# mayuelala/FollowYourClick

Measured on AMD Instinct MI355X. Metric: denoised frames/sec, 16f x 512^2 clip @ 25 DDIM steps, higher is better.
Workload: dtype bf16; 1 GPU; configs[1]: AnimationPipeline DDIM loop, SD-1.5 UNet3D + mm_sd_v15-shaped motion modules (random init), 1 clip/GPU of 16 frames 512x512, 25 DDIM steps, CFG 8.0, mask + first-frame concat, fps/flow conditioning; frames=16, height=512, width=512, ddim_steps=25, parallelism=dp1 (independent clips, weight broadcast 0.00 GiB in 0.00s)

## Files before the change

followyourclick_amd/csrc/attention.hip:

```cpp
#include "attention_kernel.h"

extern "C" int fyc_attention(const fyc_attn_args* a, void* stream) {
  FYC_REQUIRE(a && a->q && a->k && a->vt && a->o, "fyc_attention: null pointer");
  FYC_REQUIRE(g_fyc_zero_page != nullptr, "fyc_attention: fyc_init() not called");
  FYC_REQUIRE(a->dtype == FYC_BF16 || a->dtype == FYC_F16, "fyc_attention: bf16 / f16 only (f32 parity mode uses materialised attention)");
  FYC_REQUIRE(a->batch > 0 && a->heads > 0 && a->n_q > 0 && a->n_k > 0, "fyc_attention: bad sizes");
  FYC_REQUIRE(a->d % 8 == 0 && a->d >= 8 && a->d <= 160, "fyc_attention: head dim %d (multiple of 8, <= 160)", a->d);
  FYC_REQUIRE(a->ldvt % 8 == 0 && a->ldvt >= a->n_k, "fyc_attention: ldvt=%d must be a multiple of 8 and >= n_k", a->ldvt);
  FYC_REQUIRE(a->ldo % 4 == 0, "fyc_attention: ldo must be a multiple of 4");
  FYC_REQUIRE(a->kv_batch_div >= 1, "fyc_attention: kv_batch_div");
  FYC_REQUIRE(a->q_batch_mod >= 0 && a->q_batch_mod <= a->batch, "fyc_attention: q_batch_mod %d (0 .. batch)", a->q_batch_mod);
  fyca::AttnP p;
  p.q = (const bf16_t*)a->q; p.k = (const bf16_t*)a->k; p.vt = (const bf16_t*)a->vt; p.o = (bf16_t*)a->o;
  p.batch = a->batch; p.heads = a->heads; p.n_q = a->n_q; p.n_k = a->n_k; p.d = a->d; p.ldo = a->ldo; p.ldvt = a->ldvt;
  p.kv_batch_div = a->kv_batch_div; p.o_accumulate = a->o_accumulate; p.q_batch_mod = a->q_batch_mod;
  p.sl2e = a->scale * 1.44269504088896340736f; p.o_scale = a->o_scale;
  p.nqb = 0; p.zero = (const char*)g_fyc_zero_page;
  hipStream_t st = (hipStream_t)stream;
  const long long wg3 = (long long)a->batch * a->heads * ((a->n_q + 191) / 192);
  int qt = (a->n_q >= 1024 && wg3 >= 512 && a->d <= 48) ? 3 : 2;
  if (g_fyc_tuning[3] >= 2 && g_fyc_tuning[3] <= 4 && (a->d <= 80 || g_fyc_tuning[3] == 2)) qt = g_fyc_tuning[3];
  if (a->dtype == FYC_F16) {
    if (a->d <= 48) return fyca::run_small<f16_t>(p, qt, st);
    if (a->d <= 96) return fyca::run_medium<f16_t>(p, qt, st);
    return fyca::run_large<f16_t>(p, st);
  }
  if (a->d <= 48) return fyca::run_small<bf16_t>(p, qt, st);
  if (a->d <= 96) return fyca::run_medium<bf16_t>(p, qt, st);
  return fyca::run_large<bf16_t>(p, st);
}
```

followyourclick_amd/csrc/attention_kernel.h:

```cpp
#pragma once
#include <type_traits>

#include "fyc_common.h"

namespace fyca {

struct AttnP {
  const bf16_t* q; const bf16_t* k; const bf16_t* vt; bf16_t* o;
  int batch, heads, n_q, n_k, d, ldo, ldvt, kv_batch_div, o_accumulate;
  int q_batch_mod;
  float sl2e, o_scale;
  int nqb;
  const char* zero;
};

#define FYC_1 0x3F80
static __device__ __attribute__((aligned(16))) const unsigned short fyc_ones[72] = {
    FYC_1, FYC_1, FYC_1, FYC_1, FYC_1, FYC_1, FYC_1, FYC_1, FYC_1, FYC_1, FYC_1, FYC_1, FYC_1, FYC_1, FYC_1, FYC_1,
    FYC_1, FYC_1, FYC_1, FYC_1, FYC_1, FYC_1, FYC_1, FYC_1, FYC_1, FYC_1, FYC_1, FYC_1, FYC_1, FYC_1, FYC_1, FYC_1,
    FYC_1, FYC_1, FYC_1, FYC_1, FYC_1, FYC_1, FYC_1, FYC_1, FYC_1, FYC_1, FYC_1, FYC_1, FYC_1, FYC_1, FYC_1, FYC_1,
    FYC_1, FYC_1, FYC_1, FYC_1, FYC_1, FYC_1, FYC_1, FYC_1, FYC_1, FYC_1, FYC_1, FYC_1, FYC_1, FYC_1, FYC_1, FYC_1,
    FYC_1, 0, 0, 0, 0, 0, 0, 0};
#undef FYC_1
#define FYC_1 0x3C00
static __device__ __attribute__((aligned(16))) const unsigned short fyc_ones_f16[72] = {
    FYC_1, FYC_1, FYC_1, FYC_1, FYC_1, FYC_1, FYC_1, FYC_1, FYC_1, FYC_1, FYC_1, FYC_1, FYC_1, FYC_1, FYC_1, FYC_1,
    FYC_1, FYC_1, FYC_1, FYC_1, FYC_1, FYC_1, FYC_1, FYC_1, FYC_1, FYC_1, FYC_1, FYC_1, FYC_1, FYC_1, FYC_1, FYC_1,
    FYC_1, FYC_1, FYC_1, FYC_1, FYC_1, FYC_1, FYC_1, FYC_1, FYC_1, FYC_1, FYC_1, FYC_1, FYC_1, FYC_1, FYC_1, FYC_1,
    FYC_1, FYC_1, FYC_1, FYC_1, FYC_1, FYC_1, FYC_1, FYC_1, FYC_1, FYC_1, FYC_1, FYC_1, FYC_1, FYC_1, FYC_1, FYC_1,
    FYC_1, 0, 0, 0, 0, 0, 0, 0};
#undef FYC_1
template <typename T> __device__ __forceinline__ const unsigned short* ones_table();
template <> __device__ __forceinline__ const unsigned short* ones_table<bf16_t>() { return fyc_ones; }
template <> __device__ __forceinline__ const unsigned short* ones_table<f16_t>() { return fyc_ones_f16; }

typedef __attribute__((ext_vector_type(4))) short s16x4;

template <typename T> struct AttnMma;
template <> struct AttnMma<bf16_t> {
  __device__ static __forceinline__ f32x4 k32(bf16x8 a, bf16x8 b, f32x4 c) { return __builtin_amdgcn_mfma_f32_16x16x32_bf16(a, b, c, 0, 0, 0); }
  __device__ static __forceinline__ f32x4 k16(s16x4 a, s16x4 b, f32x4 c) { return __builtin_amdgcn_mfma_f32_16x16x16bf16_1k(a, b, c, 0, 0, 0); }
};
template <> struct AttnMma<f16_t> {
  __device__ static __forceinline__ f32x4 k32(f16x8 a, f16x8 b, f32x4 c) { return __builtin_amdgcn_mfma_f32_16x16x32_f16(a, b, c, 0, 0, 0); }
  __device__ static __forceinline__ f32x4 k16(s16x4 a, s16x4 b, f32x4 c) {
    return __builtin_amdgcn_mfma_f32_16x16x16f16(__builtin_bit_cast(f16x4, a), __builtin_bit_cast(f16x4, b), c, 0, 0, 0);
  }
};

__device__ __forceinline__ void glds16(const void* gsrc, char* lds_wave_base) {
  __builtin_amdgcn_global_load_lds((const __attribute__((address_space(1))) void*)gsrc,
                                   (__attribute__((address_space(3))) void*)lds_wave_base, 16, 0, 0);
}
template <int N> __device__ __forceinline__ void wait_vmcnt() { asm volatile("s_waitcnt vmcnt(%0)" ::"n"(N) : "memory"); }

#ifndef FYC_ATTN_BUILTIN_ISSUE
__device__ __forceinline__ void dma4_masked(unsigned long long m0_, unsigned long long m1_, unsigned long long m2_, unsigned long long m3_,
                                            unsigned o0, unsigned o1, unsigned o2, unsigned o3,
                                            const char* b0, const char* b1, const char* b2, const char* b3,
                                            unsigned l0, unsigned l1, unsigned l2, unsigned l3) {
  unsigned keep_m0;
  unsigned long long keep_exec;
  asm volatile("s_mov_b32 %[km0], m0\n\ts_mov_b64 %[kex], exec\n\t"
               "s_mov_b64 exec, %[ma]\n\ts_cbranch_execz 1f\n\ts_mov_b32 m0, %[la]\n\ts_nop 0\n\tglobal_load_lds_dwordx4 %[oa], %[ba]\n"
               "1:\n\ts_mov_b64 exec, %[mb]\n\ts_cbranch_execz 2f\n\ts_mov_b32 m0, %[lb]\n\ts_nop 0\n\tglobal_load_lds_dwordx4 %[ob], %[bb]\n"
               "2:\n\ts_mov_b64 exec, %[mc]\n\ts_cbranch_execz 3f\n\ts_mov_b32 m0, %[lc]\n\ts_nop 0\n\tglobal_load_lds_dwordx4 %[oc], %[bc]\n"
               "3:\n\ts_mov_b64 exec, %[md]\n\ts_cbranch_execz 4f\n\ts_mov_b32 m0, %[ld]\n\ts_nop 0\n\tglobal_load_lds_dwordx4 %[od], %[bd]\n"
               "4:\n\ts_mov_b64 exec, %[kex]\n\ts_mov_b32 m0, %[km0]"
               : [km0] "=&s"(keep_m0), [kex] "=&s"(keep_exec)
               : [ma] "s"(m0_), [mb] "s"(m1_), [mc] "s"(m2_), [md] "s"(m3_), [oa] "v"(o0), [ob] "v"(o1), [oc] "v"(o2), [od] "v"(o3),
                 [ba] "s"(b0), [bb] "s"(b1), [bc] "s"(b2), [bd] "s"(b3), [la] "s"(l0), [lb] "s"(l1), [lc] "s"(l2), [ld] "s"(l3)
               : "memory");
}
#endif

#ifdef FYC_ATTN_SETPRIO
#define FYC_ATTN_PRIO(x) __builtin_amdgcn_s_setprio(x)
#else
#define FYC_ATTN_PRIO(x) do { } while (0)
#endif

constexpr float RESCALE_THR = 6.0f;

__device__ __forceinline__ float quad_max(float mx) {
  mx = fmaxf(mx, __builtin_bit_cast(float, __builtin_amdgcn_ds_swizzle(__builtin_bit_cast(int, mx), 0x401F)));
  return swap32_max(mx);
}

template <typename T, int DP16, int DVT, int QT>
__global__ void __launch_bounds__(256, (DP16 == 3 && DVT == 3 && QT == 3) ? 3 : 1) fyc_attn_kernel(const AttnP p) {
  typedef typename Pair16<T>::Vec8 Frag;
  const unsigned short* const fyc_ones = ones_table<T>();
  constexpr int KS = DP16 / 2;
  constexpr bool TAIL = (DP16 & 1) != 0;
  constexpr bool MSUB = (DVT == DP16);
  constexpr bool PIPE = DP16 <= 3;
  constexpr int DC = DP16 * 2;
  constexpr bool KXOR = (DC == 8);
  constexpr int PC = KXOR ? 8 : DC + 1;
  constexpr int KB = 64;
  constexpr int K_IT = (KB * PC + 255) / 256, K_BYTES = K_IT * 256 * 16;
  constexpr int V_ROWS = DVT * 16, V_IT = (V_ROWS * 8 + 255) / 256, V_BYTES = V_IT * 256 * 16;
  constexpr int STAGE = K_BYTES + V_BYTES, LOADS = K_IT + V_IT, NS = 3;
  extern __shared__ __attribute__((aligned(16))) char smem[];

  const int tid = threadIdx.x, lane = tid & 63;
  const int wave = __builtin_amdgcn_readfirstlane(tid >> 6);
  const int g = lane >> 4, r16 = lane & 15;

  const int BH = p.batch * p.heads;
  int bh, qb;
  if ((BH & 7) == 0) {
    const int xcd = blockIdx.x & 7, j = blockIdx.x >> 3;
    bh = (j / p.nqb) * 8 + xcd;
    qb = j % p.nqb;
  } else {
    bh = blockIdx.x / p.nqb;
    qb = blockIdx.x % p.nqb;
  }
  const int b = bh / p.heads, h = bh - b * p.heads;
  const int kvb = (b / p.kv_batch_div) * p.heads + h;
  const int bh_q = p.q_batch_mod > 0 ? (b % p.q_batch_mod) * p.heads + h : bh;
  const T* Q = reinterpret_cast<const T*>(p.q) + (long long)bh_q * p.n_q * p.d;
  const T* K = reinterpret_cast<const T*>(p.k) + (long long)kvb * p.n_k * p.d;
  const T* VT = reinterpret_cast<const T*>(p.vt) + (long long)kvb * p.d * p.ldvt;
  const char* zero = p.zero;
  const int ntiles = (p.n_k + KB - 1) / KB;
  const int dchunks = p.d >> 3;

  constexpr bool OFFS_IN_LDS = (K_IT + V_IT) <= 4;
  constexpr unsigned NODATA = 0xffffffffu;
  unsigned k_off[K_IT], v_off[V_IT];
  int my_loads = 0;
#pragma unroll
  for (int it = 0; it < K_IT; ++it) {
    const int L = it * 256 + tid, row = L / PC, cc = L - row * PC;
    const int c = KXOR ? (cc ^ (row & 7)) : cc;
    k_off[it] = (row < KB && c < dchunks) ? (unsigned)(row * p.d + c * 8) * 2u : NODATA;
    my_loads += __builtin_amdgcn_ballot_w64(k_off[it] != NODATA) != 0 ? 1 : 0;
  }
#pragma unroll
  for (int it = 0; it < V_IT; ++it) {
    const int L = it * 256 + tid, row = L >> 3, cc = L & 7;
    const int c = cc ^ (row & 7);
    v_off[it] = (row < p.d) ? (unsigned)(row * p.ldvt + c * 8) * 2u : NODATA;
    my_loads += __builtin_amdgcn_ballot_w64(v_off[it] != NODATA) != 0 ? 1 : 0;
  }
  my_loads = __builtin_amdgcn_readfirstlane(my_loads);
#ifndef FYC_ATTN_BUILTIN_ISSUE
  unsigned long long dmask[4] = {0ull, 0ull, 0ull, 0ull};
  if (K_IT + V_IT <= 4) {
#pragma unroll
    for (int it = 0; it < K_IT; ++it) dmask[it] = __builtin_amdgcn_ballot_w64(k_off[it] != NODATA);
#pragma unroll
    for (int it = 0; it < V_IT; ++it) dmask[K_IT + it] = __builtin_amdgcn_ballot_w64(v_off[it] != NODATA);
  }
  const unsigned lds_ring = (unsigned)(size_t)(__attribute__((address_space(3))) char*)smem;
#endif
  char* const offs_lds = smem + NS * STAGE + tid * 16;
  if (OFFS_IN_LDS) {
    u32x4 o4 = {NODATA, NODATA, NODATA, NODATA};
#pragma unroll
    for (int it = 0; it < K_IT; ++it) o4[it] = k_off[it];
#pragma unroll
    for (int it = 0; it < V_IT; ++it) o4[K_IT + it] = v_off[it];
    *reinterpret_cast<u32x4*>(offs_lds) = o4;
  }
  auto issue_const = [&](int stage) {
    char* sK = smem + stage * STAGE;
    char* sV = sK + K_BYTES;
#pragma unroll
    for (int it = 0; it < K_IT; ++it) {
      const int L = it * 256 + tid, row = L / PC, cc = L - row * PC;
      const int c = KXOR ? (cc ^ (row & 7)) : cc;
      if (k_off[it] == NODATA) glds16((MSUB && row < KB && c == dchunks) ? (const void*)(fyc_ones + 64) : (const void*)zero, sK + (it * 256 + wave * 64) * 16);
    }
#pragma unroll
    for (int it = 0; it < V_IT; ++it) {
      const int row = (it * 256 + tid) >> 3;
      if (v_off[it] == NODATA) glds16(row == p.d ? (const void*)fyc_ones : (const void*)zero, sV + (it * 256 + wave * 64) * 16);
    }
  };
  auto issue_full = [&](int tile, int stage) {
    char* sK = smem + stage * STAGE;
    char* sV = sK + K_BYTES;
    const char* kb = reinterpret_cast<const char*>(K) + (long long)tile * (KB * 2) * p.d;
    const char* vb = reinterpret_cast<const char*>(VT) + (long long)tile * (KB * 2);
#ifndef FYC_ATTN_BUILTIN_ISSUE
    if constexpr (OFFS_IN_LDS) {
      const u32x4 o4 = *reinterpret_cast<const u32x4*>(offs_lds);
      const unsigned lk = lds_ring + stage * STAGE + wave * 1024, lv = lk + K_BYTES;
      auto base = [&](int i) { return i < K_IT ? kb : vb; };
      auto ldst = [&](int i) { return i < K_IT ? lk + i * 4096 : lv + (i - K_IT) * 4096; };
      dma4_masked(dmask[0], dmask[1], dmask[2], dmask[3], o4[0], o4[1], o4[2], o4[3], base(0), base(1), base(2), base(3), ldst(0), ldst(1), ldst(2), ldst(3));
      return;
    }
#endif
    unsigned ko[K_IT], vo[V_IT];
    if (OFFS_IN_LDS) {
      const u32x4 o4 = *reinterpret_cast<const u32x4*>(offs_lds);
#pragma unroll
      for (int it = 0; it < K_IT; ++it) ko[it] = o4[it];
#pragma unroll
      for (int it = 0; it < V_IT; ++it) vo[it] = o4[K_IT + it];
    } else {
#pragma unroll
      for (int it = 0; it < K_IT; ++it) ko[it] = k_off[it];
#pragma unroll
      for (int it = 0; it < V_IT; ++it) vo[it] = v_off[it];
    }
#pragma unroll
    for (int it = 0; it < K_IT; ++it)
      if (ko[it] != NODATA) glds16(kb + ko[it], sK + (it * 256 + wave * 64) * 16);
#pragma unroll
    for (int it = 0; it < V_IT; ++it)
      if (vo[it] != NODATA) glds16(vb + vo[it], sV + (it * 256 + wave * 64) * 16);
  };
  auto issue_general = [&](int tile, int stage) {
    char* sK = smem + stage * STAGE;
    char* sV = sK + K_BYTES;
    const int key0 = tile * KB;
#pragma unroll
    for (int it = 0; it < K_IT; ++it) {
      const int L = it * 256 + tid, row = L / PC, cc = L - row * PC;
      const int c = KXOR ? (cc ^ (row & 7)) : cc;
      const int key = key0 + row;
      const bool live = row < KB && key < p.n_k;
      const void* src = zero;
      if (live && c < dchunks) src = K + (long long)key * p.d + c * 8;
      else if (MSUB && live && c == dchunks) src = fyc_ones + 64;
      glds16(src, sK + (it * 256 + wave * 64) * 16);
    }
#pragma unroll
    for (int it = 0; it < V_IT; ++it) {
      const int L = it * 256 + tid, row = L >> 3, cc = L & 7;
      const int c = cc ^ (row & 7);
      const int key = key0 + c * 8;
      const void* src = zero;
      if (row < p.d) { if (key < p.ldvt) src = VT + (long long)row * p.ldvt + key; }
      else if (row == p.d) src = fyc_ones;
      glds16(src, sV + (it * 256 + wave * 64) * 16);
    }
  };
  const int nfull = p.n_k / KB;
  auto issue = [&](int tile, int stage) { if (tile < nfull) issue_full(tile, stage); else issue_general(tile, stage); };
  auto loads_of = [&](int tile) { return tile < nfull ? my_loads : LOADS; };
  auto wait_dyn = [&](int n) {
    switch (n) {
      case 0: wait_vmcnt<0>(); break;   case 1: wait_vmcnt<1>(); break;   case 2: wait_vmcnt<2>(); break;   case 3: wait_vmcnt<3>(); break;
      case 4: wait_vmcnt<4>(); break;   case 5: wait_vmcnt<5>(); break;   case 6: wait_vmcnt<6>(); break;   case 7: wait_vmcnt<7>(); break;
      case 8: wait_vmcnt<8>(); break;   case 9: wait_vmcnt<9>(); break;   case 10: wait_vmcnt<10>(); break; case 11: wait_vmcnt<11>(); break;
      default: wait_vmcnt<12>(); break;
    }
  };
  static_assert(LOADS <= 12, "wait_dyn covers up to 12 DMA instructions per tile");
#pragma unroll
  for (int st = 0; st < NS; ++st) issue_const(st);
  issue(0, 0);
  if (ntiles > 1) issue(1, 1);

  const int qbase = qb * (64 * QT) + wave * (16 * QT);
  Frag qf[QT][KS > 0 ? KS : 1];
  s16x4 qt4[QT];
#pragma unroll
  for (int qt = 0; qt < QT; ++qt) {
    const int query = qbase + qt * 16 + r16;
    const bool qok = query < p.n_q;
#pragma unroll
    for (int ks = 0; ks < KS; ++ks) {
      const int dd = 32 * ks + 8 * g;
      float v[8];
      load8<T>((qok && dd < p.d) ? Q + (long long)query * p.d + dd : reinterpret_cast<const T*>(zero), v);
      u32x4 pk;
#pragma unroll
      for (int i = 0; i < 4; ++i) pk[i] = Pair16<T>::pack(v[2 * i] * p.sl2e, v[2 * i + 1] * p.sl2e);
      qf[qt][ks] = __builtin_bit_cast(Frag, pk);
    }
    if (TAIL) {
      const int dd = 32 * KS + 4 * g;
      float v[4];
      ElemIO<T>::ld4((qok && dd < p.d) ? Q + (long long)query * p.d + dd : reinterpret_cast<const T*>(zero), v);
      u32x2 pk = {Pair16<T>::pack(v[0] * p.sl2e, v[1] * p.sl2e), Pair16<T>::pack(v[2] * p.sl2e, v[3] * p.sl2e)};
      qt4[qt] = __builtin_bit_cast(s16x4, pk);
    }
  }
  constexpr int MOFF = MSUB ? ((DP16 * 16 - 8) - (TAIL ? 32 * KS : 32 * (KS - 1))) : 0;
  constexpr int MG = TAIL ? MOFF / 4 : MOFF / 8;
  auto set_neg_max = [&](int qt, float m_bf16_exact) {
    const unsigned short bits = Pair16<T>::to_bits(-m_bf16_exact);
    if (g == MG) {
      if (TAIL) qt4[qt][0] = (short)bits;
      else {
        u32x4 t = __builtin_bit_cast(u32x4, qf[qt][KS > 0 ? KS - 1 : 0]);
        t[0] = (t[0] & 0xffff0000u) | bits;
        qf[qt][KS > 0 ? KS - 1 : 0] = __builtin_bit_cast(Frag, t);
      }
    }
  };

  f32x4 o[QT][DVT];
  float m_run[QT];
#pragma unroll
  for (int qt = 0; qt < QT; ++qt) {
    m_run[qt] = 0.f;
#pragma unroll
    for (int dv = 0; dv < DVT; ++dv) o[qt][dv] = (f32x4){0.f, 0.f, 0.f, 0.f};
  }
  bool started = false;

  int st_c = 0, st_i = (ntiles > 1) ? 2 : 1;
  auto tile_body = [&](const int tile, auto steady_c) __attribute__((always_inline)) {
    constexpr bool STEADY = decltype(steady_c)::value;
    if (STEADY && my_loads == LOADS) wait_vmcnt<LOADS>();
    else if (STEADY) wait_dyn(my_loads);
    else wait_dyn(tile + 1 < ntiles ? loads_of(tile + 1) : 0);
    __builtin_amdgcn_s_barrier();
    if (STEADY) { issue_full(tile + 2, st_i); st_i = (st_i + 1 == NS) ? 0 : st_i + 1; }
    else if (tile + 2 < ntiles) { issue(tile + 2, st_i); st_i = (st_i + 1 == NS) ? 0 : st_i + 1; }
    const char* sK = smem + st_c * STAGE;
    const char* sV = sK + K_BYTES;
    st_c = (st_c + 1 == NS) ? 0 : st_c + 1;
    const bool tail = STEADY ? false : (tile * KB + KB > p.n_k);
    auto qk = [&](int kb, f32x4 (&s)[2][QT]) {
      const char* kr[2];
#pragma unroll
      for (int t = 0; t < 2; ++t) kr[t] = sK + (kb * 32 + 8 * (r16 >> 2) + 4 * t + (r16 & 3)) * (PC * 16);
      s16x4 kt4[2];
      if (TAIL) {
#pragma unroll
        for (int t = 0; t < 2; ++t) {
          const int krow = kb * 32 + 8 * (r16 >> 2) + 4 * t + (r16 & 3);
          const int chunk = 4 * KS + (g >> 1);
          kt4[t] = *reinterpret_cast<const s16x4*>(kr[t] + (KXOR ? (chunk ^ (krow & 7)) : chunk) * 16 + (g & 1) * 8);
        }
      }
      FYC_ATTN_PRIO(1);
#pragma unroll
      for (int t = 0; t < 2; ++t)
#pragma unroll
        for (int qt = 0; qt < QT; ++qt) {
          s[t][qt] = (f32x4){0.f, 0.f, 0.f, 0.f};
          if (TAIL) s[t][qt] = AttnMma<T>::k16(kt4[t], qt4[qt], s[t][qt]);
        }
      if (TAIL && KS > 0) __builtin_amdgcn_sched_barrier(0);
#pragma unroll
      for (int t = 0; t < 2; ++t) {
        const int krow = kb * 32 + 8 * (r16 >> 2) + 4 * t + (r16 & 3);
        Frag kf[KS > 0 ? KS : 1];
#pragma unroll
        for (int ks = 0; ks < KS; ++ks) {
          const int chunk = 4 * ks + g;
          kf[ks] = *reinterpret_cast<const Frag*>(kr[t] + (KXOR ? (chunk ^ (krow & 7)) : chunk) * 16);
        }
#pragma unroll
        for (int qt = 0; qt < QT; ++qt)
#pragma unroll
          for (int ks = 0; ks < KS; ++ks) s[t][qt] = AttnMma<T>::k32(kf[ks], qf[qt][ks], s[t][qt]);
      }
      FYC_ATTN_PRIO(0);
    };
    auto softmax_pv = [&](int kb, f32x4 (&s)[2][QT], f32x4 (&sn)[2][QT], bool has_next) {
      float mx[QT];
#pragma unroll
      for (int qt = 0; qt < QT; ++qt) {
        if (tail) {
#pragma unroll
          for (int t = 0; t < 2; ++t)
#pragma unroll
            for (int r = 0; r < 4; ++r)
              if (tile * KB + kb * 32 + 8 * g + 4 * t + r >= p.n_k) s[t][qt][r] = -INFINITY;
        }
        const float m0 = fmaxf(fmaxf(s[0][qt][0], s[0][qt][1]), s[0][qt][2]);
        const float m1 = fmaxf(fmaxf(s[0][qt][3], s[1][qt][0]), s[1][qt][1]);
        mx[qt] = fmaxf(fmaxf(m0, m1), fmaxf(s[1][qt][2], s[1][qt][3]));
      }
      bool move = !started;
#pragma unroll
      for (int qt = 0; qt < QT; ++qt) move = move || (MSUB ? mx[qt] > RESCALE_THR : mx[qt] > m_run[qt] + RESCALE_THR);
      float shift[QT];
#pragma unroll
      for (int qt = 0; qt < QT; ++qt) shift[qt] = MSUB ? 0.f : m_run[qt];
      if (__builtin_amdgcn_ballot_w64(move) != 0) {
#pragma unroll
        for (int qt = 0; qt < QT; ++qt) mx[qt] = quad_max(mx[qt]);
#pragma unroll
        for (int qt = 0; qt < QT; ++qt) {
          const bool mv = !started || (MSUB ? mx[qt] > RESCALE_THR : mx[qt] > m_run[qt] + RESCALE_THR);
          if (MSUB) {
            const float m_new = mv ? round_through<T>(m_run[qt] + mx[qt]) : m_run[qt];
            const float delta = m_new - m_run[qt];
            const float alpha = started ? __builtin_amdgcn_exp2f(-delta) : 1.0f;
            m_run[qt] = m_new;
            shift[qt] = delta;
            set_neg_max(qt, m_new);
            if (has_next) {
#pragma unroll
              for (int t = 0; t < 2; ++t)
#pragma unroll
                for (int r = 0; r < 4; ++r) sn[t][qt][r] -= delta;
            }
#pragma unroll
            for (int dv = 0; dv < DVT; ++dv) { o[qt][dv][0] *= alpha; o[qt][dv][1] *= alpha; o[qt][dv][2] *= alpha; o[qt][dv][3] *= alpha; }
          } else {
            const float m_new = mv ? mx[qt] : m_run[qt];
            const float alpha = started ? __builtin_amdgcn_exp2f(m_run[qt] - m_new) : 1.0f;
            m_run[qt] = m_new;
            shift[qt] = m_new;
#pragma unroll
            for (int dv = 0; dv < DVT; ++dv) { o[qt][dv][0] *= alpha; o[qt][dv][1] *= alpha; o[qt][dv][2] *= alpha; o[qt][dv][3] *= alpha; }
          }
        }
        started = true;
#pragma unroll
        for (int qt = 0; qt < QT; ++qt)
#pragma unroll
          for (int t = 0; t < 2; ++t)
#pragma unroll
            for (int r = 0; r < 4; ++r) s[t][qt][r] -= shift[qt];
      } else if (!MSUB) {
#pragma unroll
        for (int qt = 0; qt < QT; ++qt)
#pragma unroll
          for (int t = 0; t < 2; ++t)
#pragma unroll
            for (int r = 0; r < 4; ++r) s[t][qt][r] -= shift[qt];
      }
      Frag pf[QT];
#pragma unroll
      for (int qt = 0; qt < QT; ++qt) {
        u32x4 pk;
#pragma unroll
        for (int t = 0; t < 2; ++t) {
          pk[2 * t] = Pair16<T>::pack(__builtin_amdgcn_exp2f(s[t][qt][0]), __builtin_amdgcn_exp2f(s[t][qt][1]));
          pk[2 * t + 1] = Pair16<T>::pack(__builtin_amdgcn_exp2f(s[t][qt][2]), __builtin_amdgcn_exp2f(s[t][qt][3]));
        }
        pf[qt] = __builtin_bit_cast(Frag, pk);
      }
      FYC_ATTN_PRIO(1);
#pragma unroll
      for (int dv = 0; dv < DVT; ++dv) {
        const int vrow = dv * 16 + r16;
        const int chunk = kb * 4 + g;
        const Frag vf = *reinterpret_cast<const Frag*>(sV + vrow * 128 + ((chunk ^ (vrow & 7)) * 16));
#pragma unroll
        for (int qt = 0; qt < QT; ++qt) o[qt][dv] = AttnMma<T>::k32(vf, pf[qt], o[qt][dv]);
      }
      FYC_ATTN_PRIO(0);
    };
    const int nb = STEADY ? 2 : ((tile * KB + 32 < p.n_k) ? 2 : 1);
    f32x4 s0[2][QT], s1[2][QT];
    if constexpr (PIPE) {
      qk(0, s0);
      if (nb > 1) { qk(1, s1); __builtin_amdgcn_sched_barrier(0); }
      softmax_pv(0, s0, s1, nb > 1);
      if (nb > 1) softmax_pv(1, s1, s0, false);
    } else {
      qk(0, s0);
      softmax_pv(0, s0, s1, false);
      if (nb > 1) { qk(1, s0); softmax_pv(1, s0, s1, false); }
    }
  };
  const int n_steady = nfull > 2 ? nfull - 2 : 0;
  int tile = 0;
#ifndef FYC_ATTN_ONE_LOOP
  for (; tile < n_steady; ++tile) tile_body(tile, std::true_type());
#endif
  for (; tile < ntiles; ++tile) tile_body(tile, std::false_type());

  const int lsrc = ((p.d & 15) >> 2) * 16 + r16;
#pragma unroll
  for (int qt = 0; qt < QT; ++qt) {
    const float l = __shfl(o[qt][DVT - 1][0], lsrc);
    const float inv = 1.0f / l;
    const int query = qbase + qt * 16 + r16;
    if (query >= p.n_q) continue;
    T* orow = reinterpret_cast<T*>(p.o) + ((long long)b * p.n_q + query) * p.ldo + h * p.d;
#pragma unroll
    for (int dv = 0; dv < DVT; ++dv) {
      const int dd = dv * 16 + 4 * g;
      if (dd >= p.d) continue;
      float v[4] = {o[qt][dv][0] * inv, o[qt][dv][1] * inv, o[qt][dv][2] * inv, o[qt][dv][3] * inv};
      if (p.o_accumulate) {
        float prev[4];
        ElemIO<T>::ld4(orow + dd, prev);
#pragma unroll
        for (int r = 0; r < 4; ++r) v[r] = prev[r] + p.o_scale * v[r];
      }
      ElemIO<T>::st4(orow + dd, v);
    }
  }
}

template <typename T, int DP16, int DVT, int QT>
int launch_attn(const AttnP& p0, hipStream_t st) {
  constexpr int DC = DP16 * 2;
  constexpr int PC = (DC == 8) ? 8 : DC + 1;
  constexpr int K_BYTES = ((64 * PC + 255) / 256) * 256 * 16;
  constexpr int V_BYTES = ((DVT * 16 * 8 + 255) / 256) * 256 * 16;
  constexpr int smem = 3 * (K_BYTES + V_BYTES) + 256 * 16;
  static_assert(smem <= 160 * 1024, "LDS budget");
  auto kern = fyc_attn_kernel<T, DP16, DVT, QT>;
  (void)hipFuncSetAttribute(reinterpret_cast<const void*>(kern), hipFuncAttributeMaxDynamicSharedMemorySize, smem);
  AttnP p = p0;
  p.nqb = (p.n_q + 64 * QT - 1) / (64 * QT);
  dim3 grid(p.batch * p.heads * p.nqb);
  hipLaunchKernelGGL(kern, grid, dim3(256), smem, st, p);
  FYC_CHECK_LAUNCH("fyc_attention");
  return 0;
}

template <typename T> int run_small(const AttnP& p, int qt, hipStream_t st);
template <typename T> int run_medium(const AttnP& p, int qt, hipStream_t st);
template <typename T> int run_large(const AttnP& p, hipStream_t st);

#define FYC_ATTN_CASE(D, QT) case D: return launch_attn<T, (D + 15) / 16, D / 16 + 1, QT>(p, st)

}
```

Before: 14.33 frames/s.

## Add KV-resident multi-query-block attention mode and lazy softmax rescale checks

Adds a RESIDENT kernel variant: when n_k fits in the three LDS stages (≤192 keys, e.g. text cross-attention), each workgroup loads K/V^T once and loops over several query blocks. This is meant to cut repeated K/V DMA traffic and launch overhead. The steady-state softmax loop also changes. It does one wave-wide max check per tile pair, uses inline-asm in-place updates and a peeled first steady tile, and uses a finer wait_own vmcnt wait. These add complexity and register-pressure risk.

```diff
diff --git a/followyourclick_amd/csrc/attention.hip b/followyourclick_amd/csrc/attention.hip
--- a/followyourclick_amd/csrc/attention.hip
+++ b/followyourclick_amd/csrc/attention.hip
@@ -15,11 +15,14 @@
   p.batch = a->batch; p.heads = a->heads; p.n_q = a->n_q; p.n_k = a->n_k; p.d = a->d; p.ldo = a->ldo; p.ldvt = a->ldvt;
   p.kv_batch_div = a->kv_batch_div; p.o_accumulate = a->o_accumulate; p.q_batch_mod = a->q_batch_mod;
   p.sl2e = a->scale * 1.44269504088896340736f; p.o_scale = a->o_scale;
-  p.nqb = 0; p.zero = (const char*)g_fyc_zero_page;
+  p.nqb = 0; p.resident = 0; p.qb_per = 1; p.nchunk = 0; p.zero = (const char*)g_fyc_zero_page;
   hipStream_t st = (hipStream_t)stream;
   const long long wg3 = (long long)a->batch * a->heads * ((a->n_q + 191) / 192);
   int qt = (a->n_q >= 1024 && wg3 >= 512 && a->d <= 48) ? 3 : 2;
-  if (g_fyc_tuning[3] >= 2 && g_fyc_tuning[3] <= 4 && (a->d <= 80 || g_fyc_tuning[3] == 2)) qt = g_fyc_tuning[3];
+  const int t3 = g_fyc_tuning[3];
+  const int tune_qt = (t3 >= 16 && t3 < 48) ? (t3 & 15) : t3;
+  if (tune_qt >= 2 && tune_qt <= 4 && (a->d <= 80 || tune_qt == 2)) qt = tune_qt;
+  p.resident = (t3 >= 16 && t3 < 32) ? 0 : (t3 >= 32 && t3 < 48) ? 2 : 1;
   if (a->dtype == FYC_F16) {
     if (a->d <= 48) return fyca::run_small<f16_t>(p, qt, st);
     if (a->d <= 96) return fyca::run_medium<f16_t>(p, qt, st);
diff --git a/followyourclick_amd/csrc/attention_kernel.h b/followyourclick_amd/csrc/attention_kernel.h
--- a/followyourclick_amd/csrc/attention_kernel.h
+++ b/followyourclick_amd/csrc/attention_kernel.h
@@ -11,6 +11,8 @@
   int q_batch_mod;
   float sl2e, o_scale;
   int nqb;
+  int resident;
+  int qb_per, nchunk;
   const char* zero;
 };
 
@@ -53,6 +55,13 @@
                                    (__attribute__((address_space(3))) void*)lds_wave_base, 16, 0, 0);
 }
 template <int N> __device__ __forceinline__ void wait_vmcnt() { asm volatile("s_waitcnt vmcnt(%0)" ::"n"(N) : "memory"); }
+template <int L> __device__ __forceinline__ void wait_own(int mine) {
+  static_assert(L >= 2, "K and V^T are at least one DMA instruction each");
+  asm volatile("s_waitcnt vmcnt(%1)\n\ts_cmp_ge_u32 %0, %1\n\ts_cbranch_scc1 1f\n\t"
+               "s_waitcnt vmcnt(%2)\n\ts_cmp_ge_u32 %0, %2\n\ts_cbranch_scc1 1f\n\t"
+               "s_waitcnt vmcnt(%3)\n1:"
+               :: "s"(mine), "n"(L), "n"(L - 1), "n"(L - 2) : "memory", "scc");
+}
 
 #ifndef FYC_ATTN_BUILTIN_ISSUE
 __device__ __forceinline__ void dma4_masked(unsigned long long m0_, unsigned long long m1_, unsigned long long m2_, unsigned long long m3_,
@@ -80,6 +89,18 @@
 #define FYC_ATTN_PRIO(x) do { } while (0)
 #endif
 
+__device__ __forceinline__ void keep_reg(float& dst, float src) { asm volatile("v_mov_b32 %0, %1" : "+v"(dst) : "v"(src)); }
+__device__ __forceinline__ void keep_reg(unsigned& dst, unsigned src) { asm volatile("v_mov_b32 %0, %1" : "+v"(dst) : "v"(src)); }
+__device__ __forceinline__ void sub_in_place(f32x4& x, float y) {
+#pragma unroll
+  for (int r = 0; r < 4; ++r) { float t = x[r]; asm volatile("v_sub_f32 %0, %0, %1" : "+v"(t) : "v"(y)); x[r] = t; }
+}
+__device__ __forceinline__ void mul_in_place(f32x4& x, float y) {
+#pragma unroll
+  for (int r = 0; r < 4; ++r) { float t = x[r]; asm volatile("v_mul_f32 %0, %0, %1" : "+v"(t) : "v"(y)); x[r] = t; }
+}
+__device__ __forceinline__ void move_path_enter() { asm volatile("s_nop 7\n\ts_nop 7\n\ts_nop 3" ::: "memory"); }
+
 constexpr float RESCALE_THR = 6.0f;
 
 __device__ __forceinline__ float quad_max(float mx) {
@@ -87,7 +108,23 @@
   return swap32_max(mx);
 }
 
-template <typename T, int DP16, int DVT, int QT>
+template <int N> __device__ __forceinline__ float max_chain(const float* v) {
+  float acc = v[0];
+#pragma unroll
+  for (int i = 1; i + 1 < N; i += 2) acc = fmaxf(fmaxf(acc, v[i]), v[i + 1]);
+  if ((N & 1) == 0) acc = fmaxf(acc, v[N - 1]);
+  return acc;
+}
+template <int N> __device__ __forceinline__ float max_tree(const float (&v)[N]) {
+  if constexpr (N < 16) return max_chain<N>(v);
+  else {
+    constexpr int Q = N / 4;
+    const float a = max_chain<Q>(v), b = max_chain<Q>(v + Q), c = max_chain<Q>(v + 2 * Q), d = max_chain<N - 3 * Q>(v + 3 * Q);
+    return fmaxf(fmaxf(fmaxf(a, b), c), d);
+  }
+}
+
+template <typename T, int DP16, int DVT, int QT, bool RESIDENT>
 __global__ void __launch_bounds__(256, (DP16 == 3 && DVT == 3 && QT == 3) ? 3 : 1) fyc_attn_kernel(const AttnP p) {
   typedef typename Pair16<T>::Vec8 Frag;
   const unsigned short* const fyc_ones = ones_table<T>();
@@ -104,20 +141,23 @@
   constexpr int STAGE = K_BYTES + V_BYTES, LOADS = K_IT + V_IT, NS = 3;
   extern __shared__ __attribute__((aligned(16))) char smem[];
 
-  const int tid = threadIdx.x, lane = tid & 63;
+  int tid = threadIdx.x, lane = tid & 63;
   const int wave = __builtin_amdgcn_readfirstlane(tid >> 6);
-  const int g = lane >> 4, r16 = lane & 15;
+  int g = lane >> 4, r16 = lane & 15;
 
   const int BH = p.batch * p.heads;
-  int bh, qb;
+  const int nch = RESIDENT ? p.nchunk : p.nqb;
+  int bh, qc;
   if ((BH & 7) == 0) {
     const int xcd = blockIdx.x & 7, j = blockIdx.x >> 3;
-    bh = (j / p.nqb) * 8 + xcd;
-    qb = j % p.nqb;
+    bh = (j / nch) * 8 + xcd;
+    qc = j % nch;
   } else {
-    bh = blockIdx.x / p.nqb;
-    qb = blockIdx.x % p.nqb;
-  }
+    bh = blockIdx.x / nch;
+    qc = blockIdx.x % nch;
+  }
+  const int qb0 = RESIDENT ? qc * p.qb_per : qc;
+  const int qb1 = RESIDENT ? (qb0 + p.qb_per < p.nqb ? qb0 + p.qb_per : p.nqb) : qb0 + 1;
   const int b = bh / p.heads, h = bh - b * p.heads;
   const int kvb = (b / p.kv_batch_div) * p.heads + h;
   const int bh_q = p.q_batch_mod > 0 ? (b % p.q_batch_mod) * p.heads + h : bh;
@@ -255,9 +295,21 @@
   };
   static_assert(LOADS <= 12, "wait_dyn covers up to 12 DMA instructions per tile");
 #pragma unroll
-  for (int st = 0; st < NS; ++st) issue_const(st);
-  issue(0, 0);
-  if (ntiles > 1) issue(1, 1);
+  for (int st = 0; st < NS; ++st)
+    if (!RESIDENT || st < ntiles) issue_const(st);
+  if constexpr (RESIDENT) {
+#pragma unroll
+    for (int st = 0; st < NS; ++st)
+      if (st < ntiles) issue(st, st);
+    wait_vmcnt<0>();
+    __builtin_amdgcn_s_barrier();
+  } else {
+    issue(0, 0);
+    if (ntiles > 1) issue(1, 1);
+  }
+  int st_i = (ntiles > 1) ? 2 : 1;
+
+  for (int qb = qb0; qb < qb1; ++qb) {
 
   const int qbase = qb * (64 * QT) + wave * (16 * QT);
   Frag qf[QT][KS > 0 ? KS : 1];
@@ -286,15 +338,23 @@
   }
   constexpr int MOFF = MSUB ? ((DP16 * 16 - 8) - (TAIL ? 32 * KS : 32 * (KS - 1))) : 0;
   constexpr int MG = TAIL ? MOFF / 4 : MOFF / 8;
-  auto set_neg_max = [&](int qt, float m_bf16_exact) {
+  auto set_neg_max = [&](int qt, float m_bf16_exact, auto in_place_c) {
+    constexpr bool IN_PLACE = decltype(in_place_c)::value;
     const unsigned short bits = Pair16<T>::to_bits(-m_bf16_exact);
-    if (g == MG) {
-      if (TAIL) qt4[qt][0] = (short)bits;
-      else {
-        u32x4 t = __builtin_bit_cast(u32x4, qf[qt][KS > 0 ? KS - 1 : 0]);
-        t[0] = (t[0] & 0xffff0000u) | bits;
-        qf[qt][KS > 0 ? KS - 1 : 0] = __builtin_bit_cast(Frag, t);
-      }
+    if (TAIL) {
+      u32x2 t = __builtin_bit_cast(u32x2, qt4[qt]);
+      unsigned t0 = t[0];
+      const unsigned t1 = g == MG ? ((t0 & 0xffff0000u) | bits) : t0;
+      if (IN_PLACE) keep_reg(t0, t1); else t0 = t1;
+      t[0] = t0;
+      qt4[qt] = __builtin_bit_cast(s16x4, t);
+    } else {
+      u32x4 t = __builtin_bit_cast(u32x4, qf[qt][KS > 0 ? KS - 1 : 0]);
+      unsigned t0 = t[0];
+      const unsigned t1 = g == MG ? ((t0 & 0xffff0000u) | bits) : t0;
+      if (IN_PLACE) keep_reg(t0, t1); else t0 = t1;
+      t[0] = t0;
+      qf[qt][KS > 0 ? KS - 1 : 0] = __builtin_bit_cast(Frag, t);
     }
   };
 
@@ -308,15 +368,17 @@
   }
   bool started = false;
 
-  int st_c = 0, st_i = (ntiles > 1) ? 2 : 1;
-  auto tile_body = [&](const int tile, auto steady_c) __attribute__((always_inline)) {
+  int st_c = 0;
+  auto tile_body = [&](const int tile, auto steady_c, auto first_c) __attribute__((always_inline)) {
     constexpr bool STEADY = decltype(steady_c)::value;
-    if (STEADY && my_loads == LOADS) wait_vmcnt<LOADS>();
-    else if (STEADY) wait_dyn(my_loads);
-    else wait_dyn(tile + 1 < ntiles ? loads_of(tile + 1) : 0);
-    __builtin_amdgcn_s_barrier();
-    if (STEADY) { issue_full(tile + 2, st_i); st_i = (st_i + 1 == NS) ? 0 : st_i + 1; }
-    else if (tile + 2 < ntiles) { issue(tile + 2, st_i); st_i = (st_i + 1 == NS) ? 0 : st_i + 1; }
+    constexpr bool FIRST = decltype(first_c)::value;
+    if constexpr (!RESIDENT) {
+      if (STEADY) wait_own<LOADS>(my_loads);
+      else wait_dyn(tile + 1 < ntiles ? loads_of(tile + 1) : 0);
+      __builtin_amdgcn_s_barrier();
+      if (STEADY) { issue_full(tile + 2, st_i); st_i = (st_i + 1 == NS) ? 0 : st_i + 1; }
+      else if (tile + 2 < ntiles) { issue(tile + 2, st_i); st_i = (st_i + 1 == NS) ? 0 : st_i + 1; }
+    }
     const char* sK = smem + st_c * STAGE;
     const char* sV = sK + K_BYTES;
     st_c = (st_c + 1 == NS) ? 0 : st_c + 1;
@@ -359,8 +421,44 @@
       }
       FYC_ATTN_PRIO(0);
     };
-    auto softmax_pv = [&](int kb, f32x4 (&s)[2][QT], f32x4 (&sn)[2][QT], bool has_next) {
+    auto tile_moves = [&](const f32x4 (&sa)[2][QT], const f32x4 (&sb)[2][QT], auto nb_c) __attribute__((always_inline)) -> bool {
+      constexpr int NB = decltype(nb_c)::value;
+      if constexpr (MSUB) {
+        float v[NB * QT * 8];
+#pragma unroll
+        for (int b2 = 0; b2 < NB; ++b2)
+#pragma unroll
+          for (int qt = 0; qt < QT; ++qt)
+#pragma unroll
+            for (int t = 0; t < 2; ++t)
+#pragma unroll
+              for (int r = 0; r < 4; ++r) v[((b2 * QT + qt) * 2 + t) * 4 + r] = (b2 == 0 ? sa : sb)[t][qt][r];
+        return __builtin_amdgcn_ballot_w64(max_tree(v) > RESCALE_THR) != 0;
+      } else {
+        unsigned long long mv = 0;
+#pragma unroll
+        for (int qt = 0; qt < QT; ++qt) {
+          float v[NB * 8];
+#pragma unroll
+          for (int b2 = 0; b2 < NB; ++b2)
+#pragma unroll
+            for (int t = 0; t < 2; ++t)
+#pragma unroll
+              for (int r = 0; r < 4; ++r) v[(b2 * 2 + t) * 4 + r] = (b2 == 0 ? sa : sb)[t][qt][r];
+          mv |= __builtin_amdgcn_ballot_w64(max_tree(v) > m_run[qt] + RESCALE_THR);
+        }
+        return mv != 0;
+      }
+    };
+    auto softmax_pv = [&](int kb, f32x4 (&s)[2][QT], f32x4 (&sn)[2][QT], bool has_next, bool check) __attribute__((always_inline)) {
+      const bool was_started = STEADY ? !(FIRST && kb == 0) : started;
+      constexpr bool IN_PLACE = STEADY && !FIRST && PIPE;
+      auto sub4 = [&](f32x4& x, float y) { if constexpr (IN_PLACE) sub_in_place(x, y); else { x[0] -= y; x[1] -= y; x[2] -= y; x[3] -= y; } };
+      auto mul4 = [&](f32x4& x, float y) { if constexpr (IN_PLACE) mul_in_place(x, y); else { x[0] *= y; x[1] *= y; x[2] *= y; x[3] *= y; } };
+      auto set1 = [&](float& x, float y) { if constexpr (IN_PLACE) keep_reg(x, y); else x = y; };
       float mx[QT];
+      unsigned long long fire = 0;
+      if (check) {
 #pragma unroll
       for (int qt = 0; qt < QT; ++qt) {
         if (tail) {
@@ -374,56 +472,62 @@
         const float m1 = fmaxf(fmaxf(s[0][qt][3], s[1][qt][0]), s[1][qt][1]);
         mx[qt] = fmaxf(fmaxf(m0, m1), fmaxf(s[1][qt][2], s[1][qt][3]));
       }
-      bool move = !started;
-#pragma unroll
-      for (int qt = 0; qt < QT; ++qt) move = move || (MSUB ? mx[qt] > RESCALE_THR : mx[qt] > m_run[qt] + RESCALE_THR);
-      float shift[QT];
-#pragma unroll
-      for (int qt = 0; qt < QT; ++qt) shift[qt] = MSUB ? 0.f : m_run[qt];
-      if (__builtin_amdgcn_ballot_w64(move) != 0) {
+      fire = __builtin_amdgcn_ballot_w64(!was_started);
+#pragma unroll
+      for (int qt = 0; qt < QT; ++qt) fire |= __builtin_amdgcn_ballot_w64(MSUB ? mx[qt] > RESCALE_THR : mx[qt] > m_run[qt] + RESCALE_THR);
+      }
+      if (fire != 0) {
+        float shift[QT];
+        if constexpr (IN_PLACE) {
+          move_path_enter();
+          float probe = 0.f;
+#pragma unroll
+          for (int qt = 0; qt < QT; ++qt)
+#pragma unroll
+            for (int dv = 0; dv < DVT; ++dv) probe += o[qt][dv][0];
+          asm volatile("" ::"v"(probe));
+        }
 #pragma unroll
         for (int qt = 0; qt < QT; ++qt) mx[qt] = quad_max(mx[qt]);
 #pragma unroll
         for (int qt = 0; qt < QT; ++qt) {
-          const bool mv = !started || (MSUB ? mx[qt] > RESCALE_THR : mx[qt] > m_run[qt] + RESCALE_THR);
+          const bool mv = !was_started || (MSUB ? mx[qt] > RESCALE_THR : mx[qt] > m_run[qt] + RESCALE_THR);
           if (MSUB) {
             const float m_new = mv ? round_through<T>(m_run[qt] + mx[qt]) : m_run[qt];
             const float delta = m_new - m_run[qt];
-            const float alpha = started ? __builtin_amdgcn_exp2f(-delta) : 1.0f;
-            m_run[qt] = m_new;
+            const float alpha = was_started ? __builtin_amdgcn_exp2f(-delta) : 1.0f;
+            set1(m_run[qt], m_new);
             shift[qt] = delta;
-            set_neg_max(qt, m_new);
+            set_neg_max(qt, m_new, std::integral_constant<bool, IN_PLACE>());
             if (has_next) {
 #pragma unroll
-              for (int t = 0; t < 2; ++t)
-#pragma unroll
-                for (int r = 0; r < 4; ++r) sn[t][qt][r] -= delta;
+              for (int t = 0; t < 2; ++t) sub4(sn[t][qt], delta);
             }
 #pragma unroll
-            for (int dv = 0; dv < DVT; ++dv) { o[qt][dv][0] *= alpha; o[qt][dv][1] *= alpha; o[qt][dv][2] *= alpha; o[qt][dv][3] *= alpha; }
+            for (int dv = 0; dv < DVT; ++dv) mul4(o[qt][dv], alpha);
           } else {
             const float m_new = mv ? mx[qt] : m_run[qt];
-            const float alpha = started ? __builtin_amdgcn_exp2f(m_run[qt] - m_new) : 1.0f;
-            m_run[qt] = m_new;
-            shift[qt] = m_new;
-#pragma unroll
-            for (int dv = 0; dv < DVT; ++dv) { o[qt][dv][0] *= alpha; o[qt][dv][1] *= alpha; o[qt][dv][2] *= alpha; o[qt][dv][3] *= alpha; }
+            const float alpha = was_started ? __builtin_amdgcn_exp2f(m_run[qt] - m_new) : 1.0f;
+            set1(m_run[qt], m_new);
+#pragma unroll
+            for (int dv = 0; dv < DVT; ++dv) mul4(o[qt][dv], alpha);
           }
         }
-        started = true;
+        if (!STEADY) started = true;
+        if (MSUB) {
+#pragma unroll
+          for (int qt = 0; qt < QT; ++qt)
+#pragma unroll
+            for (int t = 0; t < 2; ++t) sub4(s[t][qt], shift[qt]);
+        }
+      }
+      if (!MSUB) {
 #pragma unroll
         for (int qt = 0; qt < QT; ++qt)
 #pragma unroll
           for (int t = 0; t < 2; ++t)
 #pragma unroll
-            for (int r = 0; r < 4; ++r) s[t][qt][r] -= shift[qt];
-      } else if (!MSUB) {
-#pragma unroll
-        for (int qt = 0; qt < QT; ++qt)
-#pragma unroll
-          for (int t = 0; t < 2; ++t)
-#pragma unroll
-            for (int r = 0; r < 4; ++r) s[t][qt][r] -= shift[qt];
+            for (int r = 0; r < 4; ++r) s[t][qt][r] -= m_run[qt];
       }
       Frag pf[QT];
 #pragma unroll
@@ -449,23 +553,48 @@
     };
     const int nb = STEADY ? 2 : ((tile * KB + 32 < p.n_k) ? 2 : 1);
     f32x4 s0[2][QT], s1[2][QT];
-    if constexpr (PIPE) {
+    if constexpr (STEADY && !FIRST) {
+      if constexpr (PIPE) {
+        qk(0, s0);
+        qk(1, s1);
+        __builtin_amdgcn_sched_barrier(0);
+        const bool any = tile_moves(s0, s1, std::integral_constant<int, 2>());
+        softmax_pv(0, s0, s1, true, any);
+        softmax_pv(1, s1, s0, false, any);
+      } else {
+        qk(0, s0);
+        softmax_pv(0, s0, s1, false, true);
+        qk(1, s0);
+        softmax_pv(1, s0, s1, false, true);
+      }
+    } else if constexpr (PIPE) {
       qk(0, s0);
       if (nb > 1) { qk(1, s1); __builtin_amdgcn_sched_barrier(0); }
-      softmax_pv(0, s0, s1, nb > 1);
-      if (nb > 1) softmax_pv(1, s1, s0, false);
+      softmax_pv(0, s0, s1, nb > 1, true);
+      if (nb > 1) softmax_pv(1, s1, s0, false, true);
     } else {
       qk(0, s0);
-      softmax_pv(0, s0, s1, false);
-      if (nb > 1) { qk(1, s0); softmax_pv(1, s0, s1, false); }
+      softmax_pv(0, s0, s1, false, true);
+      if (nb > 1) { qk(1, s0); softmax_pv(1, s0, s1, false, true); }
     }
   };
   const int n_steady = nfull > 2 ? nfull - 2 : 0;
   int tile = 0;
 #ifndef FYC_ATTN_ONE_LOOP
-  for (; tile < n_steady; ++tile) tile_body(tile, std::true_type());
+  if constexpr (!RESIDENT) {
+    if (n_steady > 0 && my_loads <= LOADS && my_loads + 2 >= LOADS) {
+      tile_body(0, std::true_type(), std::true_type());
+      started = true;
+      tile = 1;
+      for (; tile < n_steady; ++tile) tile_body(tile, std::true_type(), std::false_type());
+      asm volatile("" : "+v"(tid));
+      lane = tid & 63;
+      g = lane >> 4;
+      r16 = lane & 15;
+    }
+  }
 #endif
-  for (; tile < ntiles; ++tile) tile_body(tile, std::false_type());
+  for (; tile < ntiles; ++tile) tile_body(tile, std::false_type(), std::false_type());
 
   const int lsrc = ((p.d & 15) >> 2) * 16 + r16;
 #pragma unroll
@@ -489,20 +618,40 @@
       ElemIO<T>::st4(orow + dd, v);
     }
   }
+  }
 }
 
 template <typename T, int DP16, int DVT, int QT>
 int launch_attn(const AttnP& p0, hipStream_t st) {
+  constexpr int NS_HOST = 3, KB_HOST = 64;
   constexpr int DC = DP16 * 2;
   constexpr int PC = (DC == 8) ? 8 : DC + 1;
   constexpr int K_BYTES = ((64 * PC + 255) / 256) * 256 * 16;
   constexpr int V_BYTES = ((DVT * 16 * 8 + 255) / 256) * 256 * 16;
   constexpr int smem = 3 * (K_BYTES + V_BYTES) + 256 * 16;
   static_assert(smem <= 160 * 1024, "LDS budget");
-  auto kern = fyc_attn_kernel<T, DP16, DVT, QT>;
-  (void)hipFuncSetAttribute(reinterpret_cast<const void*>(kern), hipFuncAttributeMaxDynamicSharedMemorySize, smem);
   AttnP p = p0;
   p.nqb = (p.n_q + 64 * QT - 1) / (64 * QT);
+  p.qb_per = 1;
+  p.nchunk = p.nqb;
+  if (p.resident && p.n_k <= NS_HOST * KB_HOST && p.nqb >= (p.resident == 2 ? 2 : 3)) {
+    const long long total = (long long)p.batch * p.heads * p.nqb;
+    long long per = p.resident == 2 ? 3 : (total + 640) / 1280;
+    per = per > 6 ? 6 : per;
+    if (per >= 2) {
+      p.nchunk = (p.nqb + (int)per - 1) / (int)per;
+      p.qb_per = (p.nqb + p.nchunk - 1) / p.nchunk;
+    }
+  }
+  if (p.qb_per >= 2) {
+    auto kern = fyc_attn_kernel<T, DP16, DVT, QT, true>;
+    (void)hipFuncSetAttribute(reinterpret_cast<const void*>(kern), hipFuncAttributeMaxDynamicSharedMemorySize, smem);
+    hipLaunchKernelGGL(kern, dim3(p.batch * p.heads * p.nchunk), dim3(256), smem, st, p);
+    FYC_CHECK_LAUNCH("fyc_attention");
+    return 0;
+  }
+  auto kern = fyc_attn_kernel<T, DP16, DVT, QT, false>;
+  (void)hipFuncSetAttribute(reinterpret_cast<const void*>(kern), hipFuncAttributeMaxDynamicSharedMemorySize, smem);
   dim3 grid(p.batch * p.heads * p.nqb);
   hipLaunchKernelGGL(kern, grid, dim3(256), smem, st, p);
   FYC_CHECK_LAUNCH("fyc_attention");
```

Result: no change. 14.41 frames/s, median of 6 (+0.6%).
